# fallenshock/SinDDM

Hardware: AMD Instinct MI355X
Metric: diffusion steps/sec (finest scale) + imgs/sec full multi-scale sample, 1/2/4/8 GPU (higher is better)
Workload: dtype f32 (3x3 convs: binary16 hi/lo split products -- Winograd-domain GEMMs with all 4 MFMA terms, fp32 accumulate; fp32-equivalent, error vs float64 = the fp32 oracle's: tests/test_gpu_h2.py; everything else fp32); 1 GPU; C3: 6-scale pyramid, T=1000, finest scale 411x512, batch 64 per GPU, dim=160; batch_per_gpu=64, global_batch=64, scale=5, parallelism=independent chains over 1 GPU(s), one all-gather of the images

## Files before the change

sinddm_amd/csrc/conv_wh.h:

```cpp
#pragma once
#include <utility>
#include "split16.h"

namespace sinddm {

template <class F, int... I>
__device__ __forceinline__ void wh_static_for_impl(F&& f, std::integer_sequence<int, I...>) {
    (f(std::integral_constant<int, I>{}), ...);
}
template <int N, class F>
__device__ __forceinline__ void wh_static_for(F&& f) {
    wh_static_for_impl(f, std::make_integer_sequence<int, N>{});
}

#ifndef WH_ABL
#define WH_ABL 0
#endif
#ifndef WH_MIXLO
#define WH_MIXLO 1
#endif
#ifndef WH_NT
#define WH_NT 6
#endif
#ifdef WH_TIMING
__device__ unsigned long long g_wh_seg[8 * 256 * 8 * 32];
#define WH_SEG(slot) do { if (j == 2) g_wh_seg[((p.mtp * 256 + blockIdx.x) * 8 + wv) * 32 + (slot)] = __builtin_amdgcn_s_memtime(); } while (0)
#else
#define WH_SEG(slot) do {} while (0)
#endif
constexpr int WH_TH = 8, WH_TW = 32;
constexpr int WH_RS = 40;
constexpr int WH_PS = 408;
constexpr int WH_RAW = 16 * WH_PS * 4;
constexpr int WH_V = 24 * 2 * 64 * 16;
constexpr int WH_XS = 36;
constexpr int WH_X = 24 * 16 * WH_XS * 4;
constexpr int WH_LDS = 160 * 1024;
constexpr int WH_REGION = WH_LDS - WH_RAW;
constexpr int WH_VB = WH_REGION - WH_V;
static_assert(WH_X <= WH_VB && WH_V + WH_X <= WH_REGION && WH_VB % 16 == 0, "exchange buffer beside either V buffer");
constexpr int WH_TARGET_EXP = 10;
constexpr int WH_COB = 80;

inline bool wh_shape_ok(int cin, int cout) { return cin >= 32 && cin % 16 == 0 && cout % WH_COB == 0; }
inline long long wh_image_halfs(int cin, int cout) { return (long long)(cout / WH_COB) * (cin / 16) * 24 * 5 * 512; }

__device__ __forceinline__ int wh_shift_for(float m, int target) {
    const unsigned bits = __float_as_uint(m) & 0x7fffffffu;
    const int e = (int)(bits >> 23);
    if (e == 0 || e == 255) return 0;
    int s = target - (e - 127);
    return s > 100 ? 100 : (s < -100 ? -100 : s);
}

__device__ __forceinline__ void wh_u24(const float* __restrict__ w, long long base, int transpose, double (&u)[24]) {
    const double G2[4][3] = {{1., 0., 0.}, {.5, .5, .5}, {.5, -.5, .5}, {0., 0., 1.}};
    const double G4[6][3] = {{1. / 4, 0., 0.}, {-1. / 6, -1. / 6, -1. / 6}, {-1. / 6, 1. / 6, -1. / 6},
                             {1. / 24, 1. / 12, 1. / 6}, {1. / 24, -1. / 12, 1. / 6}, {0., 0., 1.}};
    double g[3][3];
#pragma unroll
    for (int a = 0; a < 3; ++a)
#pragma unroll
        for (int b = 0; b < 3; ++b) g[a][b] = (double)(transpose ? w[base + (2 - a) * 3 + (2 - b)] : w[base + a * 3 + b]);
#pragma unroll
    for (int i = 0; i < 4; ++i)
#pragma unroll
        for (int j = 0; j < 6; ++j) {
            double acc = 0.;
#pragma unroll
            for (int a = 0; a < 3; ++a) {
                double r = 0.;
#pragma unroll
                for (int b = 0; b < 3; ++b) r += G4[j][b] * g[a][b];
                acc += G2[i][a] * r;
            }
            u[i * 6 + j] = acc;
        }
}

__global__ __launch_bounds__(256) void wh_wscale_kernel(const float* __restrict__ w, float* __restrict__ wsinv, int cin,
                                                         int cout, int transpose) {
    const int m = blockIdx.x;
    const int M = transpose ? cin : cout, K = transpose ? cout : cin;
    float mx = 0.f;
    if (m < M)
        for (int k = threadIdx.x; k < K; k += 256) {
            double u[24];
            wh_u24(w, transpose ? ((long long)k * cin + m) * 9 : ((long long)m * cin + k) * 9, transpose, u);
#pragma unroll
            for (int f = 0; f < 24; ++f) mx = fmaxf(mx, fabsf((float)u[f]));
        }
    __shared__ float red[4];
#pragma unroll
    for (int o = 32; o > 0; o >>= 1) mx = fmaxf(mx, __shfl_xor(mx, o));
    if ((threadIdx.x & 63) == 0) red[threadIdx.x >> 6] = mx;
    __syncthreads();
    if (threadIdx.x == 0 && m < M) {
        mx = fmaxf(fmaxf(red[0], red[1]), fmaxf(red[2], red[3]));
        wsinv[m] = h2_pow2(-h2_shift_for(mx));
    }
}

__global__ __launch_bounds__(256) void wh_pack_kernel(const float* __restrict__ w, const float* __restrict__ wsinv,
                                                       _Float16* __restrict__ img, int cin, int cout, int transpose,
                                                       long long total) {
    const long long i = (long long)blockIdx.x * 256 + threadIdx.x;
    if (i >= total) return;
    const int M = transpose ? cin : cout, K = transpose ? cout : cin;
    const int nch = K / 16;
    long long r = i;
    const int e = (int)(r % 8); r /= 8;
    const int co16 = (int)(r % 16); r /= 16;
    const int kh = (int)(r % 2); r /= 2;
    const int n = (int)(r % 5); r /= 5;
    const int ch = (int)(r % nch); r /= nch;
    const int cb = (int)r;
    const int m = cb * WH_COB + n * 16 + co16;
    const int k = ch * 16 + kh * 8 + e;
    double u[24];
    if (m < M && k < K) wh_u24(w, transpose ? ((long long)k * cin + m) * 9 : ((long long)m * cin + k) * 9, transpose, u);
    else {
#pragma unroll
        for (int f = 0; f < 24; ++f) u[f] = 0.;
    }
    const double sc = m < M ? 1.0 / (double)wsinv[m] : 1.0;
#pragma unroll
    for (int f = 0; f < 24; ++f) {
        const double s = u[f] * sc;
        const _Float16 hi = (_Float16)(float)s;
        const _Float16 lo = (_Float16)(float)(s - (double)(float)hi);
        const long long o = ((((long long)(cb * nch + ch) * 24 + f) * 5 + n) * 2) * 256 + (kh * 16 + co16) * 8 + e;
        img[o] = hi;
        img[o + 256] = lo;
    }
}

inline int wh_pack_launch(const float* w, float* wsinv, void* img, int cin, int cout, int transpose, hipStream_t st) {
    const int M = transpose ? cin : cout, K = transpose ? cout : cin;
    hipLaunchKernelGGL(wh_wscale_kernel, dim3(M), dim3(256), 0, st, w, wsinv, cin, cout, transpose);
    SINDDM_LAUNCH_CHECK();
    const long long total = (long long)(M / WH_COB) * (K / 16) * 5 * 2 * 16 * 8;
    hipLaunchKernelGGL(wh_pack_kernel, dim3((unsigned)((total + 255) / 256)), dim3(256), 0, st, w, wsinv,
                       static_cast<_Float16*>(img), cin, cout, transpose, total);
    SINDDM_LAUNCH_CHECK();
    return 0;
}

__device__ __forceinline__ void wh_barrier() { asm volatile("s_waitcnt lgkmcnt(0)\n\ts_barrier" ::: "memory"); }

__device__ __forceinline__ float wh_dpp_shr2(float old, float src) {
    return __builtin_bit_cast(float, __builtin_amdgcn_update_dpp(__builtin_bit_cast(int, old), __builtin_bit_cast(int, src), 0x112, 0xf, 0xf, false));
}
__device__ __forceinline__ float wh_dpp_shl2(float old, float src) {
    return __builtin_bit_cast(float, __builtin_amdgcn_update_dpp(__builtin_bit_cast(int, old), __builtin_bit_cast(int, src), 0x102, 0xf, 0xf, false));
}

__global__ __launch_bounds__(512) void conv_wh_kernel(ConvArgs p, int items_per_xcd, int wg_per_xcd) {
    typedef __attribute__((address_space(3))) float lds_f;
    extern __shared__ __attribute__((aligned(16))) float smem[];
    unsigned char* const sbytes = reinterpret_cast<unsigned char*>(smem);
    unsigned char* const sRaw = sbytes;
    unsigned char* const sV = sbytes + WH_RAW;
    const unsigned lds0 = (unsigned)(size_t)(lds_f*)smem;

    const int tid = threadIdx.x;
    const int lane = tid & 63;
    const int wv = __builtin_amdgcn_readfirstlane(tid >> 6);
    const int l16 = lane & 15, kq = lane >> 4;
    const int H = p.H, W = p.W;
    const int HW = H * W;
    const int Wt = p.Wt > 0 ? p.Wt : W;
    const int nch = p.nch3;
    const bool big_out = __builtin_amdgcn_readfirstlane((size_t)p.B * p.Cout * HW > ((size_t)1 << 28)) != 0;
    constexpr int OOB = 0x40000000;
    const bool service_rt = wv >= 6;
    const int sv = wv - 6;

    const int t_q = lane & 1, t_tc = (lane >> 1) & 7, t_mg = (lane >> 4) & 1, t_trl = lane >> 5;
    const int t_tr = t_mg * 2 + t_trl, t_t16 = t_trl * 8 + t_tc;
    const int t_rdB = (((sv & 1) * 8 + 4 * t_q) * WH_PS + 2 * t_tr * WH_RS + 4 * t_tc + 4) * 4;
    const int t_rdE = (((sv & 1) * 8 + 4 * t_q) * WH_PS + 2 * t_tr * WH_RS + (t_tc == 7 ? 36 : 3)) * 4;
    const int t_wr0 = ((t_mg * 64 + (sv & 1) * 16 + t_t16) * 16) + t_q * 8;
    const int f0 = 4 * (service_rt ? 0 : wv);
    const int a_rd = ((kq & 1) * 16 + l16) * 16;

    const int xcd = blockIdx.x & 7, ls = blockIdx.x >> 3;
    const int tpi = p.tilesX * p.tilesY;
    struct Item { int b, y0, x0, cb; bool ok; };
    auto decode = [&](int j) {
        Item it;
        const int li = ls + j * wg_per_xcd;
        const int tl = li / p.coblks;
        it.cb = li - tl * p.coblks;
        const int tile = xcd * p.tiles_per_xcd + tl;
        it.ok = li < items_per_xcd && tile < p.ntiles;
        const int tcl = it.ok ? tile : 0;
        it.b = tcl / tpi;
        const int trm = tcl - it.b * tpi;
        const int tyi = trm / p.tilesX;
        it.y0 = tyi * WH_TH;
        it.x0 = (trm - tyi * p.tilesX) * WH_TW;
        return it;
    };
    auto stage_offsets = [&](const Item& it, int (&vo)[2]) {
#pragma unroll
        for (int ps = 0; ps < 2; ++ps) {
            const int qd = ps * 64 + lane;
            const int r = qd / 10, g = qd - r * 10;
            const int gy = it.y0 - 1 + r, gx = it.x0 - 4 + 4 * g;
            vo[ps] = (qd < 100 && gy >= 0 && gy < H && gx >= 0 && gx < W) ? (gy * W + gx) * 4 : OOB;
        }
    };
    auto role_body = [&](auto ROLE) {
    constexpr bool service = decltype(ROLE)::value;
    f32x4 stg[16];
    auto stage_load = [&](const __amdgpu_buffer_rsrc_t& rs, const int (&vo)[2], int c) {
#pragma unroll
        for (int k = 0; k < 8; ++k) {
            const int so = (c * 16 + (sv & 1) * 8 + k) * HW * 4;
            stg[2 * k] = (WH_ABL & 1) ? f32x4{0.f, 0.f, 0.f, 0.f} : __builtin_bit_cast(f32x4, __builtin_amdgcn_raw_buffer_load_b128(rs, vo[0], so, (WH_NT & 1) ? 2 : 0));
            stg[2 * k + 1] = (WH_ABL & 1) ? f32x4{0.f, 0.f, 0.f, 0.f} : __builtin_bit_cast(f32x4, __builtin_amdgcn_raw_buffer_load_b128(rs, vo[1], so, (WH_NT & 1) ? 2 : 0));
        }
    };
    auto stage_write = [&](unsigned char* raw) {
        unsigned char* dst = raw + (sv & 1) * 8 * WH_PS * 4 + lane * 16;
#pragma unroll
        for (int k = 0; k < 8; ++k) {
            *reinterpret_cast<f32x4*>(dst + k * WH_PS * 4) = stg[2 * k];
            if (lane < 36) *reinterpret_cast<f32x4*>(dst + k * WH_PS * 4 + 1024) = stg[2 * k + 1];
        }
    };
    auto in_rsrc = [&](int b) {
        return __builtin_amdgcn_make_buffer_rsrc(const_cast<float*>(p.in + (size_t)b * p.Cin * HW), 0, p.Cin * HW * 4, 0x00020000);
    };

    Item cur = decode(0);
    if (!cur.ok) return;
    int svoff[2] = {OOB, OOB};
#ifndef WH_SVC_PRIO
#define WH_SVC_PRIO 2
#endif
    if constexpr (service) __builtin_amdgcn_s_setprio(WH_SVC_PRIO);
    if constexpr (service) {
        stage_offsets(cur, svoff);
        stage_load(in_rsrc(cur.b), svoff, 0);
    }
    auto item_scale = [&](const Item& it, float& sxo, float& inv) {
        const int xs = p.amax_in ? wh_shift_for(p.amax_in[(size_t)it.b * AMAX_STRIDE], WH_TARGET_EXP) : 0;
        const float sg = (((it.x0 >> 5) + (it.y0 >> 3) + it.b) & 1) ? -1.0f : 1.0f;
        sxo = sg * h2_pow2(xs);
        inv = sg * h2_pow2(-xs);
    };
    int g = 0;
    auto vbuf = [&](int k) { return sV + ((k & 1) ? WH_VB : 0); };
    for (int j = 0;; ++j) {
        const Item nxt = decode(j + 1);
        const int cb = cur.cb, b = cur.b, y0 = cur.y0, x0 = cur.x0;
        float sx, inv_sx;
        item_scale(cur, sx, inv_sx);

        const __amdgpu_buffer_rsrc_t rsin = in_rsrc(b);

        auto transform = [&](const unsigned char* raw, unsigned char* vb, float sxv) {
            if (WH_ABL & 2) return;
            const f32x2 sx2{sxv, sxv};
            const unsigned char* rpB = raw + t_rdB;
            const unsigned char* rpE = raw + t_rdE;
            unsigned char* wp = vb + t_wr0;
            f32x2 d[2][4][6];
#pragma unroll
            for (int pr = 0; pr < 2; ++pr)
#pragma unroll
                for (int rr = 0; rr < 4; ++rr) {
                    const int o = ((2 * pr) * WH_PS + rr * WH_RS) * 4;
                    const f32x4 a4 = *reinterpret_cast<const f32x4*>(rpB + o), b4 = *reinterpret_cast<const f32x4*>(rpB + o + WH_PS * 4);
                    const float ae = *reinterpret_cast<const float*>(rpE + o), be = *reinterpret_cast<const float*>(rpE + o + WH_PS * 4);
                    d[pr][rr][0] = f32x2{wh_dpp_shr2(ae, a4[3]), wh_dpp_shr2(be, b4[3])};
                    d[pr][rr][1] = f32x2{a4[0], b4[0]}; d[pr][rr][2] = f32x2{a4[1], b4[1]};
                    d[pr][rr][3] = f32x2{a4[2], b4[2]}; d[pr][rr][4] = f32x2{a4[3], b4[3]};
                    d[pr][rr][5] = f32x2{wh_dpp_shl2(ae, a4[0]), wh_dpp_shl2(be, b4[0])};
                }
            wh_static_for<4>([&](auto II) {
                constexpr int i = decltype(II)::value;
                h16x2 hi[2][6], lo[2][6];
#pragma unroll
                for (int pr = 0; pr < 2; ++pr) {
                    f32x2 r[6];
#pragma unroll
                    for (int c = 0; c < 6; ++c)
                        r[c] = i == 0 ? d[pr][0][c] - d[pr][2][c] : i == 1 ? d[pr][1][c] + d[pr][2][c]
                             : i == 2 ? d[pr][2][c] - d[pr][1][c] : d[pr][1][c] - d[pr][3][c];
                    const f32x2 s24 = r[4] - 4.f * r[2], s13 = r[3] - 4.f * r[1];
                    const f32x2 u24 = r[4] - r[2], d31 = r[3] - r[1];
                    f32x2 v[6];
                    v[0] = 4.f * r[0] + (r[4] - 5.f * r[2]);
                    v[1] = s24 + s13;
                    v[2] = s24 - s13;
                    v[3] = u24 + 2.f * d31;
                    v[4] = u24 - 2.f * d31;
                    v[5] = 4.f * r[1] + (r[5] - 5.f * r[3]);
#pragma unroll
                    for (int j = 0; j < 6; ++j) {
                        const f32x2 sc = v[j] * sx2;
                        hi[pr][j] = __builtin_convertvector(sc, h16x2);
#if WH_MIXLO
                        lo[pr][j] = h16x2{(_Float16)__builtin_fmaf(v[j].x, sxv, -(float)hi[pr][j].x), (_Float16)__builtin_fmaf(v[j].y, sxv, -(float)hi[pr][j].y)};
#else
                        const f32x2 rem{__builtin_fmaf(v[j].x, sxv, -(float)hi[pr][j].x), __builtin_fmaf(v[j].y, sxv, -(float)hi[pr][j].y)};
                        lo[pr][j] = __builtin_convertvector(rem, h16x2);
#endif
                    }
                }
#pragma unroll
                for (int j = 0; j < 6; ++j) {
                    using h16x4 = __attribute__((ext_vector_type(4))) _Float16;
                    *reinterpret_cast<h16x4*>(wp + (i * 6 + j) * 2048) = h16x4{hi[0][j][0], hi[0][j][1], hi[1][j][0], hi[1][j][1]};
                    *reinterpret_cast<h16x4*>(wp + (i * 6 + j) * 2048 + 512) = h16x4{lo[0][j][0], lo[0][j][1], lo[1][j][0], lo[1][j][1]};
                }
            });
        };

        f32x4 acc[4][2][5];
#pragma unroll
        for (int a = 0; a < 4; ++a)
#pragma unroll
            for (int g = 0; g < 2; ++g)
#pragma unroll
                for (int n = 0; n < 5; ++n) acc[a][g][n] = f32x4{0.f, 0.f, 0.f, 0.f};
        const __amdgpu_buffer_rsrc_t rsw =
            __builtin_amdgcn_make_buffer_rsrc(const_cast<float*>(p.w3), 0, 0x7FFFFFF0, 0x00020000);
        const int wlane = lane * 16;
        const int wbase = ((cb * nch) * 24 + f0) * 5 * 1024;
        h16x8 ur[10];
        auto load_u = [&](int c, int fi, int n, int slot) {
            const int so = wbase + (c * 24 * 5 + fi * 5 + n) * 1024;
            ur[slot] = __builtin_bit_cast(h16x8, __builtin_amdgcn_raw_buffer_load_b128(rsw, wlane, so, 0));
        };
        auto multiply = [&](int c, const unsigned char* vb) {
            const unsigned char* A = vb + f0 * 2048 + a_rd;
            wh_static_for<4>([&](auto FI) {
                constexpr int fi = decltype(FI)::value;
                h16x8 ah0, ah1, al0, al1;
                ah0 = *reinterpret_cast<const h16x8*>(A + fi * 2048);
                ah1 = *reinterpret_cast<const h16x8*>(A + fi * 2048 + 1024);
                al0 = *reinterpret_cast<const h16x8*>(A + fi * 2048 + 512);
                al1 = *reinterpret_cast<const h16x8*>(A + fi * 2048 + 1024 + 512);
                wh_static_for<5>([&](auto NN) {
                    constexpr int n = decltype(NN)::value;
                    constexpr int slot = (fi & 1) * 5 + n;
                    const h16x8 u = ur[slot];
                    __builtin_amdgcn_sched_barrier(0);
                    if (WH_ABL & 8) {
                        asm volatile("" ::"v"(ah0), "v"(ah1), "v"(al0), "v"(al1), "v"(u));
                    } else {
                        acc[fi][0][n] = __builtin_amdgcn_mfma_f32_16x16x32_f16(al0, u, acc[fi][0][n], 0, 0, 0);
                        acc[fi][1][n] = __builtin_amdgcn_mfma_f32_16x16x32_f16(al1, u, acc[fi][1][n], 0, 0, 0);
                        acc[fi][0][n] = __builtin_amdgcn_mfma_f32_16x16x32_f16(ah0, u, acc[fi][0][n], 0, 0, 0);
                        acc[fi][1][n] = __builtin_amdgcn_mfma_f32_16x16x32_f16(ah1, u, acc[fi][1][n], 0, 0, 0);
                    }
                    __builtin_amdgcn_sched_barrier(0);
                    if (!(WH_ABL & 4)) {
                        if (fi < 2) load_u(c, fi + 2, n, slot);
                        else load_u(c + 1 < nch ? c + 1 : c, fi - 2, n, slot);
                    }
                    __builtin_amdgcn_sched_barrier(0);
                });
            });
        };

        const int e_t = tid & 31, e_co = tid >> 5;
        const int e_tr = e_t >> 3, e_tc = e_t & 7;
        const int ey = y0 + 2 * e_tr, ex = x0 + 4 * e_tc;
        f32x4 rsd[5][2];
        float ek[5], ebv[5];
        auto ep_operands = [&]() {
            const bool e_in = ex < W;
#pragma unroll
            for (int n = 0; n < 5; ++n) {
                const int co = cb * WH_COB + n * 16 + e_co;
                ek[n] = inv_sx * p.wsinv[co];
                ebv[n] = p.bias ? p.bias[co] : 0.0f;
#pragma unroll
                for (int pp = 0; pp < 2; ++pp) {
                    rsd[n][pp] = f32x4{0.f, 0.f, 0.f, 0.f};
                    if (p.resid && !(WH_ABL & 16) && e_in && ey + pp < H)
                        rsd[n][pp] = ((WH_NT & 2) && big_out) ? __builtin_nontemporal_load(reinterpret_cast<const f32x4*>(p.resid + ((size_t)b * p.Cout + co) * HW + (size_t)(ey + pp) * W + ex))
                                                 : *reinterpret_cast<const f32x4*>(p.resid + ((size_t)b * p.Cout + co) * HW + (size_t)(ey + pp) * W + ex);
                }
            }
        };

        WH_SEG(0);
        if constexpr (service) {
            const __amdgpu_buffer_rsrc_t rsnx = in_rsrc(nxt.ok ? nxt.b : b);
            float sxn = 0.f, inv_n = 0.f;
            if (nxt.ok) item_scale(nxt, sxn, inv_n);
            if (j == 0) {
                stage_write(sRaw);
                if (nch > 1) stage_load(rsin, svoff, 1);
                else if (nxt.ok) { stage_offsets(nxt, svoff); stage_load(rsnx, svoff, 0); }
                WH_SEG(1);
                transform(sRaw, vbuf(g), sx);
                wh_barrier();
            }
            WH_SEG(2);
            for (int c = 0; c < nch; ++c) {
                if (c + 1 < nch || nxt.ok) {
                    stage_write(sRaw);
                    if (c + 2 < nch) stage_load(rsin, svoff, c + 2);
                    else if (nxt.ok) {
                        if (c + 2 == nch) stage_offsets(nxt, svoff);
                        if (c + 2 == nch || nch > 1) stage_load(rsnx, svoff, c + 2 - nch);
                    }
                    if (c == 3) WH_SEG(24);
                    transform(sRaw, vbuf(g + c + 1), c + 1 < nch ? sx : sxn);
                    if (c == 3) WH_SEG(25);
                }
                wh_barrier();
                if (c < 12) WH_SEG(3 + c);
            }
            ep_operands();
        } else {
            wh_static_for<10>([&](auto SL) {
                constexpr int sl = decltype(SL)::value;
                load_u(0, sl / 5, sl % 5, sl);
            });
            WH_SEG(1);
            if (j == 0) wh_barrier();
            WH_SEG(2);
            for (int c = 0; c < nch; ++c) {
                multiply(c, vbuf(g + c));
                if (c == 3) WH_SEG(25);
                wh_barrier();
                if (c < 12) WH_SEG(3 + c);
            }
            ep_operands();
        }
        g += nch;
        WH_SEG(16);

        const int e_wr = ((f0 * 16 + l16) * WH_XS + 4 * kq) * 4;
        const int e_rd = (e_co * WH_XS + e_t) * 4;
        float amax = 0.f;
        WH_SEG(17);
        wh_static_for<5>([&](auto NN) {
            constexpr int n = decltype(NN)::value;
            unsigned char* X = sV + ((g & 1) ? 0 : WH_V);
            if constexpr (!service) {
#pragma unroll
                for (int fi = 0; fi < 4; ++fi)
#pragma unroll
                    for (int g = 0; g < 2; ++g)
                        *reinterpret_cast<f32x4*>(X + e_wr + fi * (16 * WH_XS * 4) + g * 64) = acc[fi][g][n];
            }
            wh_barrier();
            WH_SEG(18 + n);
            float m[24];
#pragma unroll
            for (int f = 0; f < 24; ++f) m[f] = *reinterpret_cast<const float*>(X + e_rd + f * (16 * WH_XS * 4));
            wh_barrier();
            float q[2][6];
#pragma unroll
            for (int j = 0; j < 6; ++j) {
                q[0][j] = m[j] + m[6 + j] + m[12 + j];
                q[1][j] = m[6 + j] - m[12 + j] - m[18 + j];
            }
            const int co = cb * WH_COB + n * 16 + e_co;
            const float k = ek[n];
            const float bv = ebv[n];
#pragma unroll
            for (int pp = 0; pp < 2; ++pp) {
                const float* z = q[pp];
                const float s12 = z[1] + z[2], d12 = z[1] - z[2], s34 = z[3] + z[4], d34 = z[3] - z[4];
                f32x4 v{z[0] + s12 + s34, d12 + 2.f * d34, s12 + 4.f * s34, d12 + 8.f * d34 + z[5]};
                const int y = ey + pp;
                if ((WH_ABL & 16) && v[0] != 123.456f) continue;
                if (y < H && ex < W) {
                    const size_t o = ((size_t)b * p.Cout + co) * HW + (size_t)y * W + ex;
                    v = v * k + bv;
                    if (p.out_pre) *reinterpret_cast<f32x4*>(p.out_pre + o) = v;
                    if (p.act == 1) v = gelu_erf4(v);
                    else if (p.act == 2) {
                        const f32x4 a = *reinterpret_cast<const f32x4*>(p.aux + o);
#pragma unroll
                        for (int e = 0; e < 4; ++e) v[e] *= gelu_erf_grad(a[e]);
                    }
                    v += rsd[n][pp];
                    if (ex + 4 > Wt) {
#pragma unroll
                        for (int e = 0; e < 4; ++e) v[e] = ex + e < Wt ? v[e] : 0.0f;
                    }
#pragma unroll
                    for (int e = 0; e < 4; ++e) amax = fmaxf(amax, fabsf(v[e]));
                    if ((WH_NT & 4) && big_out) __builtin_nontemporal_store(v, reinterpret_cast<f32x4*>(p.out + o));
                    else *reinterpret_cast<f32x4*>(p.out + o) = v;
                }
            }
        });
        if (p.amax_out) amax_publish(amax, p.amax_out + (size_t)b * AMAX_STRIDE);
        WH_SEG(23);
        if (!nxt.ok) break;
        cur = nxt;
    }
    };
    if (service_rt) role_body(std::true_type{});
    else role_body(std::false_type{});
}

#ifndef SINDDM_WH_MIN_ITEMS_PER_CU
#define SINDDM_WH_MIN_ITEMS_PER_CU 12
#endif
#ifndef SINDDM_WH_MIN_PIXELS
#define SINDDM_WH_MIN_PIXELS 12000
#endif
#ifndef SINDDM_CONV_WH
#define SINDDM_CONV_WH 1
#endif
inline bool conv_wh_applies(bool fp32_convs, int B, int H, int W, int cin, int cout) {
    if (!SINDDM_CONV_WH || fp32_convs || !wh_shape_ok(cin, cout) || W % 4 != 0) return false;
    if ((long long)cin * H * W * 4 >= 0x40000000LL) return false;
    if ((long long)H * W < SINDDM_WH_MIN_PIXELS) return false;
    return (long long)B * ((W + WH_TW - 1) / WH_TW) * ((H + WH_TH - 1) / WH_TH) * (cout / WH_COB) >=
           (long long)SINDDM_WH_MIN_ITEMS_PER_CU * wino2_cu_count();
}

inline int conv_wh_launch(const ConvArgs& a_in, hipStream_t st) {
    ConvArgs a = a_in;
    if (!wh_shape_ok(a.Cin, a.Cout) || a.W % 4 != 0 || !a.wsinv || (long long)a.Cin * a.H * a.W * 4 >= 0x40000000LL)
        return SINDDM_E_BADSHAPE;
    ConvProfiler& prof = conv_profiler();
    const bool rec = prof.on && prof.used < ConvProfiler::MAXREC;
    if (rec) {
        while (prof.created <= prof.used) {
            (void)hipEventCreate(&prof.ev[2 * prof.created]);
            (void)hipEventCreate(&prof.ev[2 * prof.created + 1]);
            ++prof.created;
        }
        (void)hipEventRecord(prof.ev[2 * prof.used], st);
    }
    a.nch3 = a.Cin / 16;
    a.coblks = a.Cout / WH_COB;
    a.tilesX = (a.W + WH_TW - 1) / WH_TW;
    a.tilesY = (a.H + WH_TH - 1) / WH_TH;
    a.ntiles = a.B * a.tilesX * a.tilesY;
    a.tiles_per_xcd = (a.ntiles + 7) / 8;
    const int ipx = a.tiles_per_xcd * a.coblks;
    int wpx = wino2_cu_count() / 8;
    if (wpx < 1) wpx = 1;
    if (wpx > ipx) wpx = ipx;
    static const hipError_t attr_rc = hipFuncSetAttribute(reinterpret_cast<const void*>(&conv_wh_kernel),
                                                          hipFuncAttributeMaxDynamicSharedMemorySize, WH_LDS);
    if (attr_rc != hipSuccess) return (int)attr_rc;
#ifdef WH_TIMING
    static int wh_launch_no = 0;
    a.mtp = wh_launch_no++ % 8;
#endif
    hipLaunchKernelGGL(conv_wh_kernel, dim3(wpx * 8), dim3(512), WH_LDS, st, a, ipx, wpx);
    if (rec) {
        (void)hipEventRecord(prof.ev[2 * prof.used + 1], st);
        const double fl = 2.0 * a.B * a.H * (a.Wt > 0 ? a.Wt : a.W) * (double)a.Cout * 9.0 * a.Cin;
        prof.note(1, fl, 2.0 * a.ntiles * 32.0 * 24.0 * 4.0 * (double)a.Cout * a.Cin, 8);
    }
    SINDDM_LAUNCH_CHECK();
    return 0;
}

}
```

Measured before the change: 703.3 sample-steps/s (finest scale, batch x steps/s, all GPUs).

## Reassign Winograd frequencies per wave so row transform happens in registers

Each compute wave now owns frequency rows spaced six apart (fj, fj+6, fj+12, fj+18) instead of four consecutive frequencies. That lets the first stage of the output inverse transform (combining rows) run in registers on the accumulators before the LDS exchange. The exchange buffer shrinks to two transformed rows, and the epilogue handles two output-channel groups per barrier pair, so there are 3 rounds instead of 5. This cuts LDS traffic and barriers in the epilogue. In exchange, the weight and V indexing change, so the pre-packed weight layout must match the new stride.

```diff
diff --git a/sinddm_amd/csrc/conv_wh.h b/sinddm_amd/csrc/conv_wh.h
--- a/sinddm_amd/csrc/conv_wh.h
+++ b/sinddm_amd/csrc/conv_wh.h
@@ -34,7 +34,7 @@
 constexpr int WH_RAW = 16 * WH_PS * 4;
 constexpr int WH_V = 24 * 2 * 64 * 16;
 constexpr int WH_XS = 36;
-constexpr int WH_X = 24 * 16 * WH_XS * 4;
+constexpr int WH_X = 2 * 6 * 32 * WH_XS * 4;
 constexpr int WH_LDS = 160 * 1024;
 constexpr int WH_REGION = WH_LDS - WH_RAW;
 constexpr int WH_VB = WH_REGION - WH_V;
@@ -181,7 +181,7 @@
     const int t_rdB = (((sv & 1) * 8 + 4 * t_q) * WH_PS + 2 * t_tr * WH_RS + 4 * t_tc + 4) * 4;
     const int t_rdE = (((sv & 1) * 8 + 4 * t_q) * WH_PS + 2 * t_tr * WH_RS + (t_tc == 7 ? 36 : 3)) * 4;
     const int t_wr0 = ((t_mg * 64 + (sv & 1) * 16 + t_t16) * 16) + t_q * 8;
-    const int f0 = 4 * (service_rt ? 0 : wv);
+    const int fj = service_rt ? 0 : wv;
     const int a_rd = ((kq & 1) * 16 + l16) * 16;
 
     const int xcd = blockIdx.x & 7, ls = blockIdx.x >> 3;
@@ -330,21 +330,22 @@
         const __amdgpu_buffer_rsrc_t rsw =
             __builtin_amdgcn_make_buffer_rsrc(const_cast<float*>(p.w3), 0, 0x7FFFFFF0, 0x00020000);
         const int wlane = lane * 16;
-        const int wbase = ((cb * nch) * 24 + f0) * 5 * 1024;
+        const int wbase = ((cb * nch) * 24 + fj) * 5 * 1024;
         h16x8 ur[10];
         auto load_u = [&](int c, int fi, int n, int slot) {
-            const int so = wbase + (c * 24 * 5 + fi * 5 + n) * 1024;
+            const int so = wbase + (c * 24 * 5 + fi * 30 + n) * 1024;
             ur[slot] = __builtin_bit_cast(h16x8, __builtin_amdgcn_raw_buffer_load_b128(rsw, wlane, so, 0));
         };
         auto multiply = [&](int c, const unsigned char* vb) {
-            const unsigned char* A = vb + f0 * 2048 + a_rd;
+            const unsigned char* A = vb + fj * 2048 + a_rd;
             wh_static_for<4>([&](auto FI) {
                 constexpr int fi = decltype(FI)::value;
+                constexpr int fo = fi * 6 * 2048;
                 h16x8 ah0, ah1, al0, al1;
-                ah0 = *reinterpret_cast<const h16x8*>(A + fi * 2048);
-                ah1 = *reinterpret_cast<const h16x8*>(A + fi * 2048 + 1024);
-                al0 = *reinterpret_cast<const h16x8*>(A + fi * 2048 + 512);
-                al1 = *reinterpret_cast<const h16x8*>(A + fi * 2048 + 1024 + 512);
+                ah0 = *reinterpret_cast<const h16x8*>(A + fo);
+                ah1 = *reinterpret_cast<const h16x8*>(A + fo + 1024);
+                al0 = *reinterpret_cast<const h16x8*>(A + fo + 512);
+                al1 = *reinterpret_cast<const h16x8*>(A + fo + 1024 + 512);
                 wh_static_for<5>([&](auto NN) {
                     constexpr int n = decltype(NN)::value;
                     constexpr int slot = (fi & 1) * 5 + n;
@@ -439,63 +440,77 @@
         g += nch;
         WH_SEG(16);
 
-        const int e_wr = ((f0 * 16 + l16) * WH_XS + 4 * kq) * 4;
+        const int e_wr = ((fj * 32 + l16) * WH_XS + 4 * kq) * 4;
         const int e_rd = (e_co * WH_XS + e_t) * 4;
         float amax = 0.f;
         WH_SEG(17);
-        wh_static_for<5>([&](auto NN) {
-            constexpr int n = decltype(NN)::value;
+        if constexpr (!service) {
+#pragma unroll
+            for (int mg = 0; mg < 2; ++mg)
+#pragma unroll
+                for (int n = 0; n < 5; ++n) {
+                    acc[0][mg][n] = acc[0][mg][n] + acc[1][mg][n] + acc[2][mg][n];
+                    acc[1][mg][n] = acc[1][mg][n] - acc[2][mg][n] - acc[3][mg][n];
+                }
+        }
+        wh_static_for<3>([&](auto PS) {
+            constexpr int n0 = 2 * decltype(PS)::value;
+            constexpr int nn = n0 + 2 <= 5 ? 2 : 1;
             unsigned char* X = sV + ((g & 1) ? 0 : WH_V);
             if constexpr (!service) {
 #pragma unroll
-                for (int fi = 0; fi < 4; ++fi)
-#pragma unroll
-                    for (int g = 0; g < 2; ++g)
-                        *reinterpret_cast<f32x4*>(X + e_wr + fi * (16 * WH_XS * 4) + g * 64) = acc[fi][g][n];
+                for (int r = 0; r < 2; ++r)
+#pragma unroll
+                    for (int nl = 0; nl < nn; ++nl)
+#pragma unroll
+                        for (int mg = 0; mg < 2; ++mg)
+                            *reinterpret_cast<f32x4*>(X + e_wr + (r * 6 * 32 + nl * 16) * (WH_XS * 4) + mg * 64) = acc[r][mg][n0 + nl];
             }
             wh_barrier();
-            WH_SEG(18 + n);
-            float m[24];
-#pragma unroll
-            for (int f = 0; f < 24; ++f) m[f] = *reinterpret_cast<const float*>(X + e_rd + f * (16 * WH_XS * 4));
+            WH_SEG(18 + decltype(PS)::value);
+            float q[nn][2][6];
+#pragma unroll
+            for (int nl = 0; nl < nn; ++nl)
+#pragma unroll
+                for (int r = 0; r < 2; ++r)
+#pragma unroll
+                    for (int j = 0; j < 6; ++j)
+                        q[nl][r][j] = *reinterpret_cast<const float*>(X + e_rd + ((r * 6 + j) * 32 + nl * 16) * (WH_XS * 4));
             wh_barrier();
-            float q[2][6];
-#pragma unroll
-            for (int j = 0; j < 6; ++j) {
-                q[0][j] = m[j] + m[6 + j] + m[12 + j];
-                q[1][j] = m[6 + j] - m[12 + j] - m[18 + j];
-            }
-            const int co = cb * WH_COB + n * 16 + e_co;
-            const float k = ek[n];
-            const float bv = ebv[n];
-#pragma unroll
-            for (int pp = 0; pp < 2; ++pp) {
-                const float* z = q[pp];
-                const float s12 = z[1] + z[2], d12 = z[1] - z[2], s34 = z[3] + z[4], d34 = z[3] - z[4];
-                f32x4 v{z[0] + s12 + s34, d12 + 2.f * d34, s12 + 4.f * s34, d12 + 8.f * d34 + z[5]};
-                const int y = ey + pp;
-                if ((WH_ABL & 16) && v[0] != 123.456f) continue;
-                if (y < H && ex < W) {
-                    const size_t o = ((size_t)b * p.Cout + co) * HW + (size_t)y * W + ex;
-                    v = v * k + bv;
-                    if (p.out_pre) *reinterpret_cast<f32x4*>(p.out_pre + o) = v;
-                    if (p.act == 1) v = gelu_erf4(v);
-                    else if (p.act == 2) {
-                        const f32x4 a = *reinterpret_cast<const f32x4*>(p.aux + o);
-#pragma unroll
-                        for (int e = 0; e < 4; ++e) v[e] *= gelu_erf_grad(a[e]);
+            wh_static_for<nn>([&](auto NL) {
+                constexpr int n = n0 + decltype(NL)::value;
+                const int co = cb * WH_COB + n * 16 + e_co;
+                const float k = ek[n];
+                const float bv = ebv[n];
+#pragma unroll
+                for (int pp = 0; pp < 2; ++pp) {
+                    const float* z = q[decltype(NL)::value][pp];
+                    const float s12 = z[1] + z[2], d12 = z[1] - z[2], s34 = z[3] + z[4], d34 = z[3] - z[4];
+                    f32x4 v{z[0] + s12 + s34, d12 + 2.f * d34, s12 + 4.f * s34, d12 + 8.f * d34 + z[5]};
+                    const int y = ey + pp;
+                    if ((WH_ABL & 16) && v[0] != 123.456f) continue;
+                    if (y < H && ex < W) {
+                        const size_t o = ((size_t)b * p.Cout + co) * HW + (size_t)y * W + ex;
+                        v = v * k + bv;
+                        if (p.out_pre) *reinterpret_cast<f32x4*>(p.out_pre + o) = v;
+                        if (p.act == 1) v = gelu_erf4(v);
+                        else if (p.act == 2) {
+                            const f32x4 a = *reinterpret_cast<const f32x4*>(p.aux + o);
+#pragma unroll
+                            for (int e = 0; e < 4; ++e) v[e] *= gelu_erf_grad(a[e]);
+                        }
+                        v += rsd[n][pp];
+                        if (ex + 4 > Wt) {
+#pragma unroll
+                            for (int e = 0; e < 4; ++e) v[e] = ex + e < Wt ? v[e] : 0.0f;
+                        }
+#pragma unroll
+                        for (int e = 0; e < 4; ++e) amax = fmaxf(amax, fabsf(v[e]));
+                        if ((WH_NT & 4) && big_out) __builtin_nontemporal_store(v, reinterpret_cast<f32x4*>(p.out + o));
+                        else *reinterpret_cast<f32x4*>(p.out + o) = v;
                     }
-                    v += rsd[n][pp];
-                    if (ex + 4 > Wt) {
-#pragma unroll
-                        for (int e = 0; e < 4; ++e) v[e] = ex + e < Wt ? v[e] : 0.0f;
-                    }
-#pragma unroll
-                    for (int e = 0; e < 4; ++e) amax = fmaxf(amax, fabsf(v[e]));
-                    if ((WH_NT & 4) && big_out) __builtin_nontemporal_store(v, reinterpret_cast<f32x4*>(p.out + o));
-                    else *reinterpret_cast<f32x4*>(p.out + o) = v;
-                }
-            }
+                }
+            });
         });
         if (p.amax_out) amax_publish(amax, p.amax_out + (size_t)b * AMAX_STRIDE);
         WH_SEG(23);
```

After: 723.3 sample-steps/s (finest scale, batch x steps/s, all GPUs), median of 6. 1.03x the previous value.
